# Meowuu7/equi-articulated-pose

Hardware: AMD Instinct MI355X
Metric: point-clouds/sec (4096 pts, 60 anchors) fwd+bwd (higher is better)
Workload: dtype f32; 1 GPU; 8 x 4096-pt synthetic laptop clouds per GPU, 3-block inter backbone 1->64->128->512 (NN=64,K=24,A=60), forward+backward+Adam; clouds_per_gpu=8, points=4096, anchors=60

## Files before the change

equi-articulated-pose_amd/csrc/inv_lists.hip:

```cpp
#include "common.h"

namespace {

constexpr int RT = 1024;
constexpr int MAXN = 16384;
constexpr int SORT_COMPACT = 2048;

__global__ __launch_bounds__(256) void inv_count_kernel(int per_cloud, int n, const int32_t *__restrict__ idx,
                                                        int32_t *__restrict__ counts) {
    extern __shared__ int s_hist[];
    const int bi = blockIdx.y, t = threadIdx.x;
    for (int i = t; i < n; i += 256) s_hist[i] = 0;
    __syncthreads();
    const int chunk = (per_cloud + gridDim.x - 1) / gridDim.x;
    const int beg = blockIdx.x * chunk, end = min(per_cloud, beg + chunk);
    const int32_t *src = idx + (size_t)bi * per_cloud;
    for (int e = beg + t; e < end; e += 256) {
        const int q = src[e];
        if ((unsigned)q < (unsigned)n) atomicAdd(&s_hist[q], 1);
    }
    __syncthreads();
    for (int i = t; i < n; i += 256) {
        const int v = s_hist[i];
        if (v) atomicAdd(&counts[(size_t)bi * n + i], v);
// ... 118 lines not shown
                                                          const int32_t *__restrict__ rows, const float4 *__restrict__ src,
                                                          float4 *__restrict__ dst) {
    const int bi = blockIdx.z, ci = blockIdx.y;
    const int e = blockIdx.x * 256 + threadIdx.x;
    if (e >= rcap * na4) return;
    const int r = e / na4, a = e - r * na4;
    const int q = rows[(size_t)bi * rld + r];
    float4 v = make_float4(0.f, 0.f, 0.f, 0.f);
    if (q >= 0) v = src[(((size_t)bi * c + ci) * n + q) * na4 + a];
    dst[(((size_t)bi * c + ci) * rcap + r) * na4 + a] = v;
}

__global__ __launch_bounds__(256) void rows_scatter_kernel(int c, int n, int na4, int rcap, int rld,
                                                           const int32_t *__restrict__ rows, const float4 *__restrict__ src,
                                                           float4 *__restrict__ dst) {
    const int bi = blockIdx.z, ci = blockIdx.y;
    const int e = blockIdx.x * 256 + threadIdx.x;
    if (e >= rcap * na4) return;
    const int r = e / na4, a = e - r * na4;
    const int q = rows[(size_t)bi * rld + r];
    if (q >= 0) dst[(((size_t)bi * c + ci) * n + q) * na4 + a] = src[(((size_t)bi * c + ci) * rcap + r) * na4 + a];
}

}

extern "C" int eap_inv_lists_rows(int b, int p, int n, int nn, const int32_t *idx, int32_t *counts, int32_t *rows,
                                  int32_t *off, int32_t *cnt, int32_t *n_rows, eap_stream_t stream) {
    if (b <= 0 || p <= 0 || nn <= 0 || n <= 0) return 0;
    if (n > MAXN) return eap::bad_arg("inv_lists_rows: more than 16384 support points per cloud");
    if ((long long)p * nn >= (1ll << 31)) return eap::bad_arg("inv_lists_rows: more than 2^31 entries per cloud");
    hipStream_t s = eap::S(stream);
    int e = eap::hip_fail(hipMemsetAsync(counts, 0, sizeof(int32_t) * (size_t)b * n, s), "inv_lists_rows memset");
    if (e) return e;
    const int per_cloud = p * nn;
    e = eap::run_kernel("inv_lists_rows (count)", inv_count_kernel, eap::cdiv(per_cloud, 8192), b, 1, dim3(256), sizeof(int) * n, s, per_cloud, n, idx, counts);
    if (e) return e;
    int n2 = RT;
    while (n2 < n) n2 <<= 1;
    const size_t shmem = sizeof(unsigned long long) * n2;
    return eap::run_kernel("inv_lists_rows (sort)", inv_rows_kernel, b, 1, 1, dim3(RT), shmem, s, n, n2, counts, rows, off, cnt, n_rows);
}

extern "C" int eap_inv_lists_fill(int b, int p, int n, int nn, int rcap, const int32_t *idx, const float *gx,
                                  const int32_t *rows, const int32_t *off, int32_t *ent_p, float *ent_gx,
                                  eap_stream_t stream) {
    if (b <= 0 || p <= 0 || nn <= 0 || rcap <= 0) return 0;
    if (((long long)p * nn & 3) != 0) return eap::bad_arg("inv_lists_fill: p * nn must be a multiple of 4");
    if (rcap > n) return eap::bad_arg("inv_lists_fill: rcap exceeds the number of support points");
    return eap::run_kernel("inv_lists_fill", inv_fill_kernel, rcap, b, 1, dim3(256), 0, eap::S(stream), p * nn, nn, n, n, idx, reinterpret_cast<const float4 *>(gx),
                           rows, off, ent_p, reinterpret_cast<float4 *>(ent_gx));
}

extern "C" int eap_rows_gather_f32(int b, int c, int n, int na, int rcap, int rows_ld, const int32_t *rows,
                                   const float *src, float *dst, eap_stream_t stream) {
    if (b <= 0 || c <= 0 || rcap <= 0) return 0;
    if ((na & 3) != 0) return eap::bad_arg("rows_gather: na must be a multiple of 4");
    return eap::run_kernel("rows_gather", rows_gather_kernel, eap::cdiv((long long)rcap * (na / 4), 256), c, b, dim3(256), 0, eap::S(stream), c, n, na / 4, rcap, rows_ld,
                           rows, reinterpret_cast<const float4 *>(src), reinterpret_cast<float4 *>(dst));
}

extern "C" int eap_rows_scatter_f32(int b, int c, int n, int na, int rcap, int rows_ld, const int32_t *rows,
                                    const float *src, float *dst, eap_stream_t stream) {
    if (b <= 0 || c <= 0) return 0;
    if ((na & 3) != 0) return eap::bad_arg("rows_scatter: na must be a multiple of 4");
    hipStream_t s = eap::S(stream);
    int e = eap::hip_fail(hipMemsetAsync(dst, 0, sizeof(float) * (size_t)b * c * n * na, s), "rows_scatter memset");
    if (e || rcap <= 0) return e;
    return eap::run_kernel("rows_scatter", rows_scatter_kernel, eap::cdiv((long long)rcap * (na / 4), 256), c, b, dim3(256), 0, s, c, n, na / 4, rcap, rows_ld, rows,
                           reinterpret_cast<const float4 *>(src), reinterpret_cast<float4 *>(dst));
}
```

equi-articulated-pose_amd/csrc/norm_fold.hip:

```cpp
#include <math.h>
#include <string.h>

#include "common.h"

namespace {

constexpr int WAVE = 64;

__device__ __forceinline__ double wave_sum(double v) {
#pragma unroll
    for (int m = WAVE / 2; m >= 1; m >>= 1) v += __shfl_xor(v, m, WAVE);
    return v;
}

__device__ __forceinline__ void two_row_sums(const float *__restrict__ a, const float *__restrict__ q, int parts, int lane, double &sa, double &sq) {
    sa = 0.0, sq = 0.0;
    for (int i = lane; i < parts; i += WAVE) {
        sa += (double)a[i];
        sq += (double)q[i];
    }
    sa = wave_sum(sa);
    sq = wave_sum(sq);
}

// ... 75 lines not shown
    }
}

__global__ __launch_bounds__(256) void dense_zbound_kernel(int b, int na, int rp, int p, int ldw, long cnt_stride, const float *__restrict__ colmax,
                                                           const int32_t *__restrict__ cnt, const int32_t *__restrict__ n_rows,
                                                           float *__restrict__ words) {
    const int w = blockIdx.x * blockDim.x + threadIdx.x, cloud = blockIdx.y;
    if (w >= ldw) return;
    float v = 0.f;
    if (w < na * rp / 4) {
        const int a = 4 * w / rp, r0 = 4 * w - a * rp, live = n_rows[cloud];
        const float m = colmax[(long)cloud * na + a];
#pragma unroll
        for (int j = 0; j < 4; ++j) {
            int c = r0 + j < live ? cnt[cloud * cnt_stride + r0 + j] : 0;
            c = c < 0 ? 0 : (c > p ? p : c);
            const float t = m * (float)c;
            v = j == 0 ? t : nan_max(v, t);
        }
    }
    words[(long)cloud * ldw + w] = v;
}

__global__ __launch_bounds__(256) void dense_gbound_parts_kernel(int bc, int c, int rp, int na, int ks, const float *__restrict__ W3,
                                                                 const float *__restrict__ fc4, float *__restrict__ fpart, float *__restrict__ wsum) {
    __shared__ float red[256];
    const int t = threadIdx.x, nt = blockDim.x;
    if ((int)blockIdx.x < bc) {
        const float *src = fc4 + (long)blockIdx.x * rp * na;
        const int len = rp * na;
        float m = 0.f, m1 = 0.f, m2 = 0.f, m3 = 0.f;
        int e = t;
        for (; e + 3 * nt < len; e += 4 * nt) {
            const float v0 = src[e], v1 = src[e + nt], v2 = src[e + 2 * nt], v3 = src[e + 3 * nt];
            m = nan_max(m, fabsf(v0)), m1 = nan_max(m1, fabsf(v1)), m2 = nan_max(m2, fabsf(v2)), m3 = nan_max(m3, fabsf(v3));
        }
        for (; e < len; e += nt) m = nan_max(m, fabsf(src[e]));
        m = nan_max(nan_max(m, m1), nan_max(m2, m3));
        red[t] = m;
        __syncthreads();
        if (t < na) {
            for (int g = 1; g < nt / na; ++g) m = nan_max(m, red[t + g * na]);
            fpart[(long)blockIdx.x * na + t] = m;
        }
        return;
    }
    const int oc = blockIdx.x - bc, lane = t & (WAVE - 1), wave = t / WAVE, waves = nt / WAVE;
    float m = 0.f;
    if (wave < waves)
        for (int k = wave; k < ks; k += waves) {
            const float *row = W3 + ((long)oc * ks + k) * c;
            double s = 0.0;
            for (int i = lane; i < c; i += WAVE) s += (double)fabsf(row[i]);
            m = nan_max(m, (float)wave_sum(s));
        }
    if (lane == 0 && wave < waves) red[wave] = m;
    __syncthreads();
    if (t == 0) {
        for (int g = 1; g < waves; ++g) m = nan_max(m, red[g]);
        wsum[oc] = m * 1.0001f;
    }
}

__global__ __launch_bounds__(256) void dense_gbound_kernel(int c, int na, int o, const float *__restrict__ fpart, const float *__restrict__ wsum,
                                                           float *__restrict__ bound) {
    __shared__ float red[256];
    const int t = threadIdx.x, cloud = blockIdx.x / na, a = blockIdx.x - cloud * na;
    float m = 0.f;
    for (int ch = t; ch < c; ch += 256) m = nan_max(m, fpart[((long)cloud * c + ch) * na + a]);
    red[t] = m;
    __syncthreads();
    for (int s = 128; s >= 1; s >>= 1) {
        if (t < s) red[t] = nan_max(red[t], red[t + s]);
        __syncthreads();
    }
    m = red[0];
    for (int oc = t; oc < o; oc += 256) bound[(long)blockIdx.x * o + oc] = m * wsum[oc];
}

__global__ __launch_bounds__(256) void dense_point_order_kernel(int p, int quads, const int64_t *__restrict__ order, const int4 *__restrict__ memb,
                                                                const float *__restrict__ q_xyz, int32_t *__restrict__ order32,
                                                                int4 *__restrict__ memb_out, float *__restrict__ xyz_out,
                                                                int32_t *__restrict__ pivot_pos) {
    const long i = (long)blockIdx.x * blockDim.x + threadIdx.x;
// ... 55 lines not shown
                                        const int32_t *n_rows, float *words, eap_stream_t stream) {
    if (!colmax || !cnt || !n_rows || !words) return eap::bad_arg("so3_dense_zbound: null pointer");
    if (b <= 0 || na <= 0 || rp <= 0 || p <= 0 || ldz <= 0) return eap::bad_arg("so3_dense_zbound: b, na, rp, p and ldz must be positive");
    if (rp % 4 != 0 || ldz % 4 != 0 || (long long)na * rp > ldz || cnt_stride < rp)
        return eap::bad_arg("so3_dense_zbound: rp and ldz multiples of 4, ldz >= na * rp, the row stride of cnt >= rp");
    return eap::run_kernel("so3_dense_zbound", dense_zbound_kernel, eap::cdiv(ldz / 4, 256), b, 1, dim3(256), 0, eap::S(stream), b, na, rp, p, ldz / 4,
                           (long)cnt_stride, colmax, cnt, n_rows, words);
}

extern "C" int eap_so3_dense_gplanes_bound_f32(int b, int o, int c, int na, int ks, int rp, const float *W3, const float *fc4, float *fpart,
                                               float *wsum, float *bound, eap_stream_t stream) {
    if (!W3 || !fc4 || !fpart || !wsum || !bound) return eap::bad_arg("so3_dense_gplanes_bound: null pointer");
    if (b <= 0 || o <= 0 || c <= 0 || na <= 0 || ks <= 0 || rp <= 0) return eap::bad_arg("so3_dense_gplanes_bound: every size must be positive");
    if (na > 128 || (long long)rp * na > 0x7fffffffLL || (long long)b * c > 0x7fffffffLL - o || (long long)b * na > 0x7fffffffLL)
        return eap::bad_arg("so3_dense_gplanes_bound: na <= 128, rp * na, b * c + o and b * na below 2^31");
    const int nt = 256 / na * na;
    if (int e = eap::run_kernel("so3_dense_gplanes_bound (parts)", dense_gbound_parts_kernel, (long long)b * c + o, 1, 1, dim3(nt), 0, eap::S(stream), b * c, c,
                                rp, na, ks, W3, fc4, fpart, wsum))
        return e;
    return eap::run_kernel("so3_dense_gplanes_bound", dense_gbound_kernel, (long long)b * na, 1, 1, dim3(256), 0, eap::S(stream), c, na, o, (const float *)fpart,
                           (const float *)wsum, bound);
}

extern "C" int eap_so3_dense_point_order(int b, int p, int words, const int64_t *order, const uint32_t *memb, const float *q_xyz, int32_t *order32,
                                         uint32_t *memb_out, float *xyz_out, int32_t *pivot_pos, eap_stream_t stream) {
    if (!order || !memb || !q_xyz || !order32 || !memb_out || !xyz_out || !pivot_pos) return eap::bad_arg("so3_dense_point_order: null pointer");
    if (b <= 0 || p <= 0) return eap::bad_arg("so3_dense_point_order: b and p must be positive");
    if (words != 16 && words != 32) return eap::bad_arg("so3_dense_point_order: 16 or 32 membership words per point");
    if (!aligned16(memb) || !aligned16(memb_out)) return eap::bad_arg("so3_dense_point_order: takes 16-byte aligned membership tables");
    const int quads = words / 4;
    return eap::run_kernel("so3_dense_point_order", dense_point_order_kernel, eap::cdiv((long long)p * quads, 256), b, 1, dim3(256), 0, eap::S(stream), p, quads,
                           order, reinterpret_cast<const int4 *>(memb), q_xyz, order32, reinterpret_cast<int4 *>(memb_out), xyz_out, pivot_pos);
}
```

equi-articulated-pose_amd/vgtk/_hip.py:

```python
import ctypes
import os
import re
import struct
import types
import weakref

import torch

_PKG_ROOT = os.path.abspath(os.path.join(os.path.dirname(__file__), '..'))
LIB_PATH = os.path.join(_PKG_ROOT, 'libeap_hip.so')

if not os.path.exists(LIB_PATH):
    raise ImportError(
        f'{LIB_PATH} not found: build the HIP extension first '
        '(python -c "import __graft_entry__ as g; g.build()" or make -C equi-articulated-pose_amd/csrc). '
        'This package has no CPU fallback.')

lib = ctypes.CDLL(LIB_PATH)


_HEADERS = (os.path.join(_PKG_ROOT, 'include', 'eap_hip.h'), os.path.join(os.path.dirname(_PKG_ROOT), 'include', 'eap_hip.h'))
HEADER_PATH = next((p for p in _HEADERS if os.path.exists(p)), _HEADERS[-1])

_I64 = ctypes.c_int64
# ... 706 lines not shown
         tag={'flops': 2.0 * b * o * ks * p * nn * na, 'shape': ('group_inv_perm2', b, o, p, nn, na, ks, rcap)})
    return z


def inv_lists_rows(idx, n):
    b, p, nn = idx.shape
    dev = idx.device
    counts = torch.empty(b, n, dtype=torch.int32, device=dev)
    rows, off, cnt = torch.empty_like(counts), torch.empty_like(counts), torch.empty_like(counts)
    n_rows = torch.empty(b, dtype=torch.int32, device=dev)
    call('eap_inv_lists_rows', idx, b, p, n, nn, idx, counts, rows, off, cnt, n_rows)
    return rows, off, cnt, n_rows


def inv_lists_fill(idx, gx, rows, off, rcap):
    b, p, nn = idx.shape
    n = rows.shape[1]
    ent_p = torch.empty(b, p * nn, dtype=torch.int32, device=idx.device)
    ent_gx = torch.empty(b, p * nn, 4, dtype=torch.float32, device=idx.device)
    call('eap_inv_lists_fill', idx, b, p, n, nn, int(rcap), idx, gx, rows, off, ent_p, ent_gx)
    return ent_p, ent_gx


def rows_gather(src, rows, rcap):
    b, c, n, na = src.shape
    dst = torch.empty(b, c, rcap, na, dtype=torch.float32, device=src.device)
    call('eap_rows_gather_f32', src, b, c, n, na, int(rcap), rows.stride(0), rows, src, dst)
    return dst


def rows_scatter(src, rows, n):
    b, c, rcap, na = src.shape
    dst = torch.empty(b, c, n, na, dtype=torch.float32, device=src.device)
    call('eap_rows_scatter_f32', src, b, c, n, na, int(rcap), rows.stride(0), rows, src, dst)
    return dst





def so3_dense_supported(p, na, ks, rp, o):
    return bool(abi.eap_so3_dense_supported(int(p), int(na), int(ks), int(rp), int(o)))


DENSE_MAX_ROWS = int(abi.eap_so3_dense_max_rows())
DENSE_NARROW_ROWS = 512


def _dense_wide(memb):
    return memb.shape[2] == 32
# ... 144 lines not shown
        if geo.n_rows is not None:
            rows = sum(min((int(r) + 15) & ~15, geo.rp) for r in geo.n_rows.tolist())
    return 6.0 * o * p * geo.na * geo.ks * rows


def _dense_product(direction, geo, b, o, p, ld, scale, planes, out, flops):
    call('eap_so3_dense_product_steps_f32', out, direction, b, o, p, geo.na, geo.ks, geo.rp, ld, geo.sigma, geo.n_rows, planes, scale, geo.pt, geo.kr,
         geo.mask(direction), geo.steps(direction), out, tag={'flops': flops, 'executed_f16_flops': _dense_executed_flops(geo, o, p, direction),
         'shape': ('so3_dense', direction, b, o, p, geo.na, geo.ks, geo.rp)})
    return out


def so3_dense_bwd(gy, geo, ldz=None, colmap=None, rowmax=False):
    b, o, p, na = gy.shape
    ldz = na * geo.rp if ldz is None else int(ldz)
    colmap = geo.columns(colmap)
    scale, planes = so3_dense_split(gy, rowmax=take_rowmax_hint(gy) if rowmax is False else rowmax, colmap=colmap)
    if colmap is not None:
        p = colmap.shape[1]
    z = torch.empty(b, o, geo.ks, ldz, dtype=torch.float32, device=gy.device)
    return _dense_product(0, geo, b, o, p, ldz, scale, planes, z, 2.0 * b * o * p * na * geo.ks * geo.nn)


def so3_dense_gplanes(fc4, W3, geo):
    b, c, rp, na = fc4.shape
    o = W3.shape[0] // geo.ks
    if not GPLANES or not abi.eap_so3_dense_gplanes_supported(o, c, na, geo.ks, rp):
        return None
    ft = fc4.permute(0, 3, 2, 1).contiguous()
    if NATIVE_NORM_GLUE:
        bound = so3_dense_gplanes_bound(W3, fc4, geo.ks)
    else:
        wsum = W3.abs().sum(1).view(o, geo.ks).amax(1)
        fm = fc4.abs().amax((1, 2))
        bound = (fm[:, :, None] * (wsum * 1.0001)[None, None, :]).contiguous()
    scale = torch.empty(2, b, na, o, dtype=torch.float32, device=fc4.device)
    planes = torch.empty(b * na * o * ((geo.ks * rp + 31) // 32 * 32), dtype=torch.int32, device=fc4.device)
    call('eap_so3_dense_gplanes_f32', fc4, b, o, c, na, geo.ks, rp, W3, ft, geo.n_rows, bound, scale, planes,
         tag={'flops': 0.0, 'shape': ('so3_dense_gplanes', b, o, c, na, geo.ks, rp)})
    return scale, planes


GPLANES = True


NATIVE_NORM_GLUE = True


def _f64_bits(x):
    return struct.unpack('<q', struct.pack('<d', float(x)))[0]


def norm_fold_train(ps, pq, pivot, count, gamma, beta, eps, momentum, running_mean, running_var):
    check_input(ps, pq, gamma, beta, running_mean, running_var)
    o, parts = ps.shape
    if pivot.dim() != 1 or pivot.shape[0] != o or pivot.dtype != torch.float32 or not pivot.is_cuda:
        raise RuntimeError('norm_fold_train: pivot must be a float32 device vector (any stride) of one element per channel')
    dev = ps.device
    scale, shift, beta_copy, inv_gamma = (torch.empty(o, dtype=torch.float32, device=dev) for _ in range(4))
    mean, invstd = (torch.empty(o, dtype=torch.float64, device=dev) for _ in range(2))
    call('eap_norm_fold_train_f32', ps, o, parts, max(int(pivot.stride(0)), 1), int(count), _f64_bits(eps), _f64_bits(momentum), ps, pq, pivot, gamma,
# ... 15 lines not shown
    colmax = torch.empty(b, na, dtype=torch.float32, device=dev)
    call('eap_norm_fold_bwd_f32', pg, o, parts, b, na, int(count), pg, pgx, k1, beta, inv_gamma, gmax, xmax, dgamma, dbeta, k2, k3, coef, bound, colmax)
    return dgamma, dbeta, k2, k3, coef, bound, colmax


def so3_dense_zbound(colmax, cnt, n_rows, rp, p, ldz):
    b, na = colmax.shape
    if cnt.dtype != torch.int32 or n_rows.dtype != torch.int32 or cnt.stride(1) != 1 or not n_rows.is_contiguous():
        raise RuntimeError('so3_dense_zbound: cnt and n_rows must be int32, the rows of cnt contiguous')
    words = torch.empty(b, ldz // 4, dtype=torch.float32, device=colmax.device)
    call('eap_so3_dense_zbound_f32', colmax, b, na, int(rp), int(p), int(ldz), cnt.stride(0), colmax, cnt, n_rows, words)
    return words


def so3_dense_gplanes_bound(W3, fc4, ks):
    check_input(W3, fc4)
    b, c, rp, na = fc4.shape
    o = W3.shape[0] // ks
    dev = fc4.device
    fpart = torch.empty(b, c, na, dtype=torch.float32, device=dev)
    wsum = torch.empty(o, dtype=torch.float32, device=dev)
    bound = torch.empty(b, na, o, dtype=torch.float32, device=dev)
    call('eap_so3_dense_gplanes_bound_f32', fc4, b, o, c, na, int(ks), rp, W3, fc4, fpart, wsum, bound)
    return bound


def so3_dense_point_order(order, memb, q_xyz):
    check_input(order, memb, q_xyz)
    b, p = order.shape
    order32 = torch.empty(b, p, dtype=torch.int32, device=order.device)
    memb_out, xyz_out = torch.empty_like(memb), torch.empty_like(q_xyz)
    pivot_pos = torch.empty(1, dtype=torch.int32, device=order.device)
    call('eap_so3_dense_point_order', order, b, p, memb.shape[2], order, memb, q_xyz, order32, memb_out, xyz_out, pivot_pos)
    return order32, memb_out, xyz_out, pivot_pos


def so3_dense_fwd(g, geo, p, c=0, ldg=None, out=None, col_map=None, operand=None, o=None):
    yt = _dense_fwd_yt(g, geo, p, c, ldg, operand, o)
    b, na, o = yt.shape[0], geo.na, yt.shape[2]
    if col_map is not None:
        if out is None or col_map.dtype != torch.int32 or tuple(col_map.shape) != (b, p) or not col_map.is_contiguous() or not out.is_contiguous():
            raise RuntimeError('so3_dense_fwd: col_map must be a contiguous int32 [b,p] and come with a contiguous out')
        call('eap_so3_dense_untranspose_map_f32', yt, b, o, p, na, out.shape[2], geo.columns(col_map), yt, out)
        return out
    y = torch.empty(b, o, p, na, dtype=torch.float32, device=yt.device)
    chunks = (p + 63) // 64
# ... 363 lines not shown
```

equi-articulated-pose_amd/vgtk/so3conv/functional.py:

```python
import math
import os
import weakref

import numpy as np
import torch

import vgtk
import vgtk.functional as fr
import vgtk.pc as pctk
import vgtk.spconv as zpconv
import vgtk.cuda.grouping as cuda_nn

from .. import _hip
from . import norm_fold

inter_so3conv_feat_grouping = zpconv.inter_zpconv_grouping_naive
batched_index_select = zpconv.batched_index_select
batched_index_select_other = zpconv.batched_index_select_other

MATERIALIZE_INTER_W = False

GAMMA_SIZE = 3
ROOT = vgtk.__path__[0]
Rs, R_idx, canonical_relative = fr.icosahedron_so3(GAMMA_SIZE)
# ... 954 lines not shown
    scale, shift, mean, invstd, count, slope, sync = bn
    b, o = gy.shape[0], gy.shape[1]
    gy = gy.view(b, o, -1)
    if _native_norm_bwd(gy, count, sync):
        g_bn_w, g_bn_b, k2, k3 = _hip.norm_fold_bwd(*_hip.narrow_conv_bwd_reduce(gy, x, W, scale, shift, mean, invstd, slope, partials=True), scale, count)
        return (_hip.narrow_conv_bwd_dw(gy, x, W, scale, shift, mean, invstd, k2, k3, slope) if need_w else None), g_bn_w, g_bn_b
    sg, sgx = _hip.narrow_conv_bwd_reduce(gy, x, W, scale, shift, mean, invstd, slope)
    gW = None
    if need_w:
        k2, k3 = norm_fold.backward_coefficients(scale, sg, sgx, count, True, sync)
        gW = _hip.narrow_conv_bwd_dw(gy, x, W, scale, shift, mean, invstd, k2, k3, slope)
    return gW, sgx.float(), sg.float()



def _weight_operand(W, c, ks, pad_c=None):
    o = W.shape[0]
    W2 = W.view(o, c, ks).permute(1, 0, 2).reshape(c, o * ks).contiguous()
    if pad_c is not None and pad_c != c:
        W2 = torch.cat([W2, torch.zeros(pad_c - c, o * ks, dtype=torch.float32, device=W.device)])
    return W2


def _rows_grad_from_z(z, W2, c, rp, na, ldz, anchor_major, z_bound=None, reorder=None):
    b, (pad_c, oks) = z.shape[0], W2.shape
    gFc = torch.empty(b, pad_c, ldz, dtype=torch.float32, device=z.device)
    _hip.matmul(W2, z.view(b, oks, ldz), gFc, b_bound=z_bound)
    if anchor_major:
        return gFc[:, :c, :rp * na].reshape(b, c, na, rp).transpose(2, 3)
    gFc = gFc.view(b, c, rp, na)
    return gFc if reorder is None else _hip.anchor_reorder(gFc, reorder)


def _weight_grad_rows(z, fc4, o, ks, ldz, anchor_major, reorder=None):
    b, c, rp, na = fc4.shape
    if reorder is not None:
        fc4 = _hip.anchor_reorder(fc4, reorder)
    fc = fc4.transpose(2, 3).contiguous() if anchor_major else fc4
    return _weight_grad_from_z(z, fc.view(b, c, rp * na), b, c, o, ks, rp * na, ldz)



def _backward_dense(gy, W, feats, head, geo, bn, yact, need_f, need_w):
    b, c, n, na = feats.shape
    o, ks, p, rp = W.shape[0], geo.ks, gy.shape[2], geo.rp
    if BACKWARD_LOG is not None:
        BACKWARD_LOG.append({'channels': (c, o), 'support_rows': n, 'referenced_rows_max': int(rp), 'regime': 'dense rows',
                             **({'norm': 'in the node'} if bn is not None else {})})
    ra = na * rp
    pad_c = 128 if (c == 64 and bn is not None) else c
# ... 4 lines not shown
        native = _native_norm_bwd(gy, count, sync)
        if native:
            pg, pgx, gmax, xmax = _hip.bn_act_bwd_reduce_fromy(gy, yact, beta, inv_gamma, slope, partials=True)
            g_bn_w, g_bn_b, _, _, coef, bound, colmax = _hip.norm_fold_bwd(pg, pgx, k1, count, beta, inv_gamma, gmax, xmax)
        else:
            sg, sgx, gmax, xmax = _hip.bn_act_bwd_reduce_fromy(gy, yact, beta, inv_gamma, slope)
            g_bn_w, g_bn_b = sgx.float(), sg.float()
            k2, k3 = norm_fold.backward_coefficients(k1, sg, sgx, count, True, sync)
            coef = torch.stack([k1, k2, k3, beta, inv_gamma]).contiguous()
            bound = (k1.abs()[None, :, None] * gmax + k2.abs()[None, :, None] + k3.abs()[None, :, None] * xmax).contiguous()
        z = _hip.so3_dense_bwd_bn(gy, yact, geo, ldz, coef, bound, slope)
        if ldz % 4 == 0 and rp % 4 == 0 and native:
            z_bound = (_hip.so3_dense_zbound(colmax, head.cnt, head.n_rows, rp, p, ldz).view(torch.int32), 4, 1.0)
        elif ldz % 4 == 0 and rp % 4 == 0:
            live = torch.arange(rp, device=gy.device)[None, :] < head.n_rows[:, None]
            cntf = torch.where(live, head.cnt[:, :rp], torch.zeros_like(head.cnt[:, :rp])).clamp(min=0, max=p).to(torch.float32)
            cols = bound.amax(1)[:, :, None] * cntf[:, None, :]
            words = torch.zeros(b, ldz // 4, dtype=torch.float32, device=gy.device)
            words[:, :ra // 4] = cols.view(b, na, rp // 4, 4).amax(3).view(b, ra // 4)
            z_bound = (words.view(torch.int32), 4, 1.0)
    else:
        z = _hip.so3_dense_bwd(gy, geo, ldz)
    if need_f:
        gFr = _rows_grad_from_z(z, _weight_operand(W, c, ks, pad_c), c, rp, na, ldz, True, z_bound)
        gF = _hip.rows_scatter(gFr.contiguous(), head.rows, n)
    if need_w:
        gW = _weight_grad_rows(z, _hip.rows_gather(feats, head.rows, rp), o, ks, ldz, True)
    return gF, gW, g_bn_w, g_bn_b


def _backward_dense_parts(gy, W, feats, head, pd, need_f, need_w):
    b, c, n, na = feats.shape
    o, ks, rp = W.shape[0], pd.ks, pd.rp
    ra = na * rp
    if BACKWARD_LOG is not None:
        BACKWARD_LOG.append({'channels': (c, o), 'support_rows': n, 'referenced_rows_max': int(rp), 'regime': 'dense rows', 'parts': pd.parts.n})
    ldz = _hip.dense_pitch(ra) if (c % 128 == 0 and (o * ks) % 16 == 0 and need_f) else ra
    W2 = _weight_operand(W, c, ks) if need_f else None
    fc0 = _hip.rows_gather(feats, head.rows, rp) if need_w else None
    gFr = gW = None
    rowmax = _hip.take_rowmax_hint(gy)
    for i, geo in enumerate(pd.geo):
        perm = pd.perm[i]
        z = _hip.so3_dense_bwd(gy, geo, ldz, colmap=pd.parts.col_map[i], rowmax=rowmax)
        pe = None if perm is None else perm[:, None].expand(b, c, rp, na)
        if need_f:
            t = _rows_grad_from_z(z, W2, c, rp, na, ldz, True)
            if gFr is None:
                gFr = torch.zeros(b, c, rp, na, dtype=torch.float32, device=gy.device)
            if pe is None:
# ... 762 lines not shown
```

include/eap_hip.h:

```cpp
#ifndef EAP_HIP_H
#define EAP_HIP_H

#include <stdint.h>

#ifdef __cplusplus
extern "C" {
#endif

typedef void *eap_stream_t;

const char *eap_last_error(void);
int eap_launch_dims_ok(int64_t gx, int64_t gy, int64_t gz, int bx, int by, int bz);
const char *eap_last_kernel(void);
int eap_abi_version(void);


int eap_ball_query_f32(int b, int n, int m, float radius, int nsample, const float *new_xyz,
                       const float *xyz, int32_t *idx, eap_stream_t stream);
int eap_ball_query_f64(int b, int n, int m, float radius, int nsample, const double *new_xyz,
                       const double *xyz, int32_t *idx, eap_stream_t stream);

int eap_furthest_point_sampling_f32(int b, int n, int m, const float *xyz, float *temp,
                                    int32_t *idx, eap_stream_t stream);
int eap_furthest_point_sampling_f64(int b, int n, int m, const double *xyz, double *temp,
// ... 145 lines not shown
int eap_so3_inter_group_inv_f32(int b, int o, int p, int nn, int na, int ks, int rcap, float sigma,
                                const float *gy, const int32_t *rows, const int32_t *off,
                                const int32_t *cnt, const int32_t *ent_p, const float *ent_gx,
                                const float *rk, const uint8_t *multinv, const float *anchors,
                                int identity_anchor, float *z, eap_stream_t stream);
int eap_anchor_reorder_f32(int64_t rows, int na, const float *src, const uint8_t *order, float *dst, eap_stream_t stream);
int eap_anchor_reorder_clouds_f32(int b, int64_t rows_per_cloud, int na, const float *src, const uint8_t *order,
                                  const int32_t *nonident, float *dst, eap_stream_t stream);
int eap_so3_inter_group_inv_coset_f32(int b, int o, int p, int nn, int na, int ks, int rcap, float sigma,
                                      const float *gy, const int32_t *rows, const int32_t *off, const int32_t *cnt,
                                      const int32_t *ent_p, const float *ent_gx, const float *rk, const uint8_t *multinv,
                                      const float *anchors, int identity_anchor, const uint8_t *coset_order,
                                      const uint8_t *coset_code, float *z, eap_stream_t stream);

int eap_inv_lists_rows(int b, int p, int n, int nn, const int32_t *idx, int32_t *counts, int32_t *rows,
                       int32_t *off, int32_t *cnt, int32_t *n_rows, eap_stream_t stream);
int eap_inv_lists_fill(int b, int p, int n, int nn, int rcap, const int32_t *idx, const float *gx,
                       const int32_t *rows, const int32_t *off, int32_t *ent_p, float *ent_gx,
                       eap_stream_t stream);
int eap_rows_gather_f32(int b, int c, int n, int na, int rcap, int rows_ld, const int32_t *rows,
                        const float *src, float *dst, eap_stream_t stream);
int eap_rows_scatter_f32(int b, int c, int n, int na, int rcap, int rows_ld, const int32_t *rows,
                         const float *src, float *dst, eap_stream_t stream);

int eap_so3_dense_supported(int p, int na, int ks, int rp, int o);
int eap_so3_dense_member(int b, int p, int n, int nn, int rp, int rows_ld, const int32_t *idx, const int32_t *rows,
                         const int32_t *n_rows, int32_t *slot_of, uint32_t *memb, int32_t *flags, eap_stream_t stream);
int64_t eap_so3_dense_mask_words(int b, int p, int ks, int rp, int dir);
int eap_so3_dense_masks(int b, int p, int ks, int rp, int dir, const uint32_t *memb, uint64_t *mask, eap_stream_t stream);
int eap_so3_dense_tables_f32(int b, int p, int n, int na, int ks, int rp, int rows_ld, float sigma, const float *q_xyz,
                             const float *s_xyz, const int32_t *rows, const float *rk, const float *row_rot, float *centre, float *pt,
                             float *kr, eap_stream_t stream);
int eap_so3_dense_split_f32(int b, int m, int l, int na, int seg, int64_t seg_pitch, int mapped, const int32_t *n_rows, const uint32_t *rowmax,
                            const int32_t *colmap, const float *src, float *scale, void *planes, eap_stream_t stream);
int eap_so3_dense_product_f32(int dir, int b, int o, int p, int na, int ks, int rp, int64_t ldz, float sigma, const int32_t *n_rows, const void *planes,
                              const float *scale,
                              const float *pt, const float *kr, const uint64_t *mask, float *out, eap_stream_t stream);
int eap_so3_dense_untranspose_f32(int b, int o, int p, int na, const float *yt, float *y, float *psum, float *psq, eap_stream_t stream);
int eap_so3_dense_untranspose_map_f32(int b, int o, int p, int na, int p_dst, const int32_t *map, const float *yt, float *y,
                                      eap_stream_t stream);
int eap_so3_dense_untranspose_map_stats_f32(int b, int o, int p, int na, int p_dst, const int32_t *map, const int32_t *pivot_pos, const float *yt,
                                            float *y, float *psum, float *psq, eap_stream_t stream);
int eap_so3_dense_split_bn_f32(int b, int m, int l, int l_src, int na, const uint32_t *rowbound, const int32_t *colmap, const float *grad,
                               const float *act, const float *coef, float slope, float *scale, void *planes, eap_stream_t stream);
int eap_so3_dense_untranspose_bnact_f32(int b, int o, int p, int na, int p_dst, const int32_t *map, const float *yt, const float *bn_scale,
                                        const float *bn_shift, float slope, float *y, eap_stream_t stream);
// ... 189 lines not shown

int eap_narrow_conv_segments(int64_t n);
int eap_narrow_conv_stats_f32(int b, int o, int ck, int64_t n, const float *W, const float *x, float *pivot, float *psum, float *psq,
                              eap_stream_t stream);
int eap_narrow_conv_bnact_fwd_f32(int b, int o, int ck, int64_t n, float slope, const float *W, const float *x, const float *scale,
                                  const float *shift, float *y, eap_stream_t stream);
int eap_narrow_conv_bwd_reduce_f32(int b, int o, int ck, int64_t n, float slope, const float *gy, const float *x, const float *W,
                                   const float *scale, const float *shift, const float *mean, const float *invstd, float *pg, float *pgx,
                                   eap_stream_t stream);
int eap_narrow_conv_bwd_dw_f32(int b, int o, int ck, int64_t n, float slope, const float *gy, const float *x, const float *W,
                               const float *scale, const float *shift, const float *mean, const float *invstd, const float *k2,
                               const float *k3, float *partial, float *dW, eap_stream_t stream);

int eap_norm_fold_train_f32(int o, int parts, int64_t pivot_stride, int64_t count, int64_t eps_bits, int64_t momentum_bits, const float *ps,
                            const float *pq, const float *pivot, const float *gamma, const float *beta, float *running_mean, float *running_var,
                            float *scale, float *shift, double *mean, double *invstd, float *beta_copy, float *inv_gamma, eap_stream_t stream);
int eap_norm_fold_bwd_f32(int o, int parts, int b, int na, int64_t count, const float *pg, const float *pgx, const float *k1, const float *beta,
                          const float *inv_gamma, const float *gmax, const float *xmax, float *dgamma, float *dbeta, float *k2, float *k3, float *coef,
                          float *bound, float *colmax, eap_stream_t stream);
int eap_so3_dense_zbound_f32(int b, int na, int rp, int p, int ldz, int64_t cnt_stride, const float *colmax, const int32_t *cnt,
                             const int32_t *n_rows, float *words, eap_stream_t stream);
int eap_so3_dense_gplanes_bound_f32(int b, int o, int c, int na, int ks, int rp, const float *W3, const float *fc4, float *fpart, float *wsum,
                                    float *bound, eap_stream_t stream);
int eap_so3_dense_point_order(int b, int p, int words, const int64_t *order, const uint32_t *memb, const float *q_xyz, int32_t *order32,
                              uint32_t *memb_out, float *xyz_out, int32_t *pivot_pos, eap_stream_t stream);

int eap_anchor_attn_pool_fwd_f32(int b, int c, int n, int na, float temperature, const float *x, const float *logits,
                                 float *out, float *conf, eap_stream_t stream);
int eap_anchor_attn_pool_bwd_f32(int b, int c, int n, int na, float temperature, const float *x, const float *logits,
                                 const float *g, float *dx, float *dlogits, eap_stream_t stream);
int eap_slot_masked_mean_fwd_f32(int b, int ns, int c, int n, int na, const float *x, const float *mask,
                                 const float *inv_den, float *out, eap_stream_t stream);
int eap_slot_masked_mean_bwd_f32(int b, int ns, int c, int n, int na, const float *g, const float *mask,
                                 const float *inv_den, float *dx, eap_stream_t stream);
int eap_masked_max_fwd_f32(int b, int c, int n, int na, const float *x, const float *mask, float *out, int32_t *arg,
                           eap_stream_t stream);
int eap_masked_max_bwd_f32(int b, int c, int n, int na, const float *g, const int32_t *arg, const float *mask, float *dx,
                           eap_stream_t stream);
int eap_anchor_attn_pool_wide_fwd_f32(int b, int c, int n, int na, float temperature, const float *x, const float *logits,
                                      float *out, float *conf, eap_stream_t stream);
int eap_anchor_attn_pool_wide_bwd_f32(int b, int c, int n, int na, float temperature, const float *x, const float *logits,
                                      const float *g, float *dx, float *dlogits, eap_stream_t stream);
int eap_slot_masked_mean_wide_fwd_f32(int b, int ns, int c, int n, int na, const float *x, const float *mask,
                                      const float *inv_den, float *out, eap_stream_t stream);
int eap_slot_masked_mean_wide_bwd_f32(int b, int ns, int c, int n, int na, const float *g, const float *mask,
                                      const float *inv_den, float *dx, eap_stream_t stream);
// ... 70 lines not shown
```

Before: 173.4 point-clouds/sec.

## Gather and scatter support rows directly in anchor-major layout in dense backward

```diff
diff --git a/equi-articulated-pose_amd/csrc/inv_lists.hip b/equi-articulated-pose_amd/csrc/inv_lists.hip
--- a/equi-articulated-pose_amd/csrc/inv_lists.hip
+++ b/equi-articulated-pose_amd/csrc/inv_lists.hip
@@ -164,6 +164,78 @@
     if (q >= 0) dst[(((size_t)bi * c + ci) * n + q) * na4 + a] = src[(((size_t)bi * c + ci) * rcap + r) * na4 + a];
 }
 
+constexpr int ROWS_TILE = 64;
+
+struct DivStep {
+    int q, r, dq, dr, d;
+    __device__ __forceinline__ DivStep(int e0, int d_) : q(e0 / d_), r(e0 - (e0 / d_) * d_), dq(256 / d_), dr(256 - (256 / d_) * d_), d(d_) {}
+    __device__ __forceinline__ void next() {
+        q += dq; r += dr;
+        if (r >= d) { r -= d; ++q; }
+    }
+};
+
+__device__ __forceinline__ void tile_put4(float *t, const float4 &v) { t[0] = v.x; t[1] = v.y; t[2] = v.z; t[3] = v.w; }
+__device__ __forceinline__ float4 tile_get4(const float *t) { return make_float4(t[0], t[1], t[2], t[3]); }
+
+__global__ __launch_bounds__(256) void rows_gather_am_kernel(int c, int n, int na, int rcap, int rld, const int32_t *__restrict__ rows,
+                                                             const float *__restrict__ src, float *__restrict__ dst) {
+    extern __shared__ float rows_tile[];
+    const int bi = blockIdx.z, ci = blockIdx.y, r0 = blockIdx.x * ROWS_TILE, nr = min(ROWS_TILE, rcap - r0), pitch = na + 1, na4 = na >> 2;
+    const float *s = src + ((size_t)bi * c + ci) * n * na;
+    DivStep i(threadIdx.x, na4);
+    for (int e = threadIdx.x; e < nr * na4; e += 256, i.next()) {
+        const int q = rows[(size_t)bi * rld + r0 + i.q];
+        float4 v = make_float4(0.f, 0.f, 0.f, 0.f);
+        if ((unsigned)q < (unsigned)n) v = reinterpret_cast<const float4 *>(s + (size_t)q * na)[i.r];
+        tile_put4(rows_tile + i.q * pitch + 4 * i.r, v);
+    }
+    __syncthreads();
+    float *d = dst + ((size_t)bi * c + ci) * na * rcap + r0;
+    for (int e = threadIdx.x; e < na * ROWS_TILE; e += 256) {
+        const int a = e / ROWS_TILE, rr = e - a * ROWS_TILE;
+        if (rr < nr) d[(size_t)a * rcap + rr] = rows_tile[rr * pitch + a];
+    }
+}
+
+__global__ __launch_bounds__(256) void rows_scatter_am_kernel(int c, int n, int na, int rcap, int rld, long long sB, long long ld,
+                                                              const int32_t *__restrict__ rows, const float *__restrict__ src,
+                                                              float *__restrict__ dst) {
+    extern __shared__ float rows_tile[];
+    const int bi = blockIdx.z, ci = blockIdx.y, r0 = blockIdx.x * ROWS_TILE, nr = min(ROWS_TILE, rcap - r0), pitch = na + 1, na4 = na >> 2;
+    const float *s = src + (size_t)bi * sB + (size_t)ci * ld + r0;
+    for (int e = threadIdx.x; e < na * ROWS_TILE; e += 256) {
+        const int a = e / ROWS_TILE, rr = e - a * ROWS_TILE;
+        if (rr < nr) rows_tile[rr * pitch + a] = s[(size_t)a * rcap + rr];
+    }
+    __syncthreads();
+    float *d = dst + ((size_t)bi * c + ci) * n * na;
+    DivStep i(threadIdx.x, na4);
+    for (int e = threadIdx.x; e < nr * na4; e += 256, i.next()) {
+        const int q = rows[(size_t)bi * rld + r0 + i.q];
+        if ((unsigned)q < (unsigned)n) reinterpret_cast<float4 *>(d + (size_t)q * na)[i.r] = tile_get4(rows_tile + i.q * pitch + 4 * i.r);
+    }
+}
+
+__global__ __launch_bounds__(256) void rows_gather_ft_kernel(int c, int n, int na, int rcap, int rld, const int32_t *__restrict__ rows,
+                                                             const float *__restrict__ src, float *__restrict__ dst) {
+    extern __shared__ float rows_tile[];
+    const int bi = blockIdx.y, r = blockIdx.x, pitch = na + 1, na4 = na >> 2;
+    const int q = rows[(size_t)bi * rld + r];
+    const bool live = (unsigned)q < (unsigned)n;
+    const float *s = src + ((size_t)bi * c * n + (live ? q : 0)) * na;
+    DivStep i(threadIdx.x, na4);
+    for (int e = threadIdx.x; e < c * na4; e += 256, i.next()) {
+        float4 v = make_float4(0.f, 0.f, 0.f, 0.f);
+        if (live) v = reinterpret_cast<const float4 *>(s + (size_t)i.q * n * na)[i.r];
+        tile_put4(rows_tile + i.q * pitch + 4 * i.r, v);
+    }
+    __syncthreads();
+    float *d = dst + ((size_t)bi * na * rcap + r) * c;
+    DivStep o(threadIdx.x, c);
+    for (int e = threadIdx.x; e < na * c; e += 256, o.next()) d[(size_t)o.q * rcap * c + o.r] = rows_tile[o.r * pitch + o.q];
+}
+
 }
 
 extern "C" int eap_inv_lists_rows(int b, int p, int n, int nn, const int32_t *idx, int32_t *counts, int32_t *rows,
@@ -201,6 +273,41 @@
                            rows, reinterpret_cast<const float4 *>(src), reinterpret_cast<float4 *>(dst));
 }
 
+extern "C" int eap_rows_gather_layout_f32(int b, int c, int n, int na, int rcap, int rows_ld, int layout, const int32_t *rows,
+                                          const float *src, float *dst, eap_stream_t stream) {
+    if (layout < 0 || layout > 2) return eap::bad_arg("rows_gather_layout: layout must be 0 ([b,c,rcap,na]), 1 ([b,c,na,rcap]) or 2 ([b,na,rcap,c])");
+    if (b <= 0 || c <= 0 || rcap <= 0) return 0;
+    if (rows == nullptr || src == nullptr || dst == nullptr) return eap::bad_arg("rows_gather_layout: null pointer");
+    if (n <= 0 || na <= 0 || (na & 3) != 0 || rows_ld < rcap) return eap::bad_arg("rows_gather_layout: n and na must be positive, na a multiple of 4, rows_ld >= rcap");
+    if (!eap::aligned16(src)) return eap::bad_arg("rows_gather_layout: src must be 16-byte aligned (its rows are read as 16-byte pieces)");
+    if (layout == 0) return eap_rows_gather_f32(b, c, n, na, rcap, rows_ld, rows, src, dst, stream);
+    if (layout == 1)
+        return eap::run_kernel("rows_gather (anchor-major)", rows_gather_am_kernel, eap::cdiv(rcap, ROWS_TILE), c, b, dim3(256), sizeof(float) * ROWS_TILE * (na + 1),
+                               eap::S(stream), c, n, na, rcap, rows_ld, rows, src, dst);
+    const size_t lds = sizeof(float) * (size_t)c * (na + 1);
+    if (lds > 64 * 1024) return eap::bad_arg("rows_gather_layout: layout 2 takes c * (na + 1) <= 16384 floats (one support row in LDS)");
+    return eap::run_kernel("rows_gather (channel-innermost)", rows_gather_ft_kernel, rcap, b, 1, dim3(256), lds, eap::S(stream), c, n, na, rcap, rows_ld, rows, src,
+                           dst);
+}
+
+extern "C" int eap_rows_scatter_am_f32(int b, int c, int n, int na, int rcap, int rows_ld, int64_t src_batch, int64_t src_ld, const int32_t *rows,
+                                       const float *src, float *dst, eap_stream_t stream) {
+    if (b <= 0 || c <= 0) return 0;
+    if (dst == nullptr) return eap::bad_arg("rows_scatter_am: null pointer");
+    if (n <= 0 || na <= 0 || (na & 3) != 0) return eap::bad_arg("rows_scatter_am: n and na must be positive, na a multiple of 4");
+    if (!eap::aligned16(dst)) return eap::bad_arg("rows_scatter_am: dst must be 16-byte aligned (its rows are written as 16-byte pieces)");
+    hipStream_t s = eap::S(stream);
+    if (rcap > 0) {
+        if (rows == nullptr || src == nullptr) return eap::bad_arg("rows_scatter_am: null pointer");
+        if (rows_ld < rcap || src_ld < (int64_t)na * rcap || (src_ld & 3) != 0 || src_batch < (int64_t)c * src_ld)
+            return eap::bad_arg("rows_scatter_am: rows_ld >= rcap, src_ld >= na * rcap and a multiple of 4, src_batch >= c * src_ld");
+    }
+    int e = eap::hip_fail(hipMemsetAsync(dst, 0, sizeof(float) * (size_t)b * c * n * na, s), "rows_scatter_am memset");
+    if (e || rcap <= 0) return e;
+    return eap::run_kernel("rows_scatter (anchor-major)", rows_scatter_am_kernel, eap::cdiv(rcap, ROWS_TILE), c, b, dim3(256), sizeof(float) * ROWS_TILE * (na + 1), s, c,
+                           n, na, rcap, rows_ld, (long long)src_batch, (long long)src_ld, rows, src, dst);
+}
+
 extern "C" int eap_rows_scatter_f32(int b, int c, int n, int na, int rcap, int rows_ld, const int32_t *rows,
                                     const float *src, float *dst, eap_stream_t stream) {
     if (b <= 0 || c <= 0) return 0;
diff --git a/equi-articulated-pose_amd/csrc/norm_fold.hip b/equi-articulated-pose_amd/csrc/norm_fold.hip
--- a/equi-articulated-pose_amd/csrc/norm_fold.hip
+++ b/equi-articulated-pose_amd/csrc/norm_fold.hip
@@ -121,6 +121,25 @@
     words[(long)cloud * ldw + w] = v;
 }
 
+__device__ __forceinline__ void gbound_wsum(int oc, int c, int ks, const float *__restrict__ W3, float *__restrict__ wsum, float *red) {
+    const int t = threadIdx.x, nt = blockDim.x;
+    const int lane = t & (WAVE - 1), wave = t / WAVE, waves = nt / WAVE;
+    float m = 0.f;
+    if (wave < waves)
+        for (int k = wave; k < ks; k += waves) {
+            const float *row = W3 + ((long)oc * ks + k) * c;
+            double s = 0.0;
+            for (int i = lane; i < c; i += WAVE) s += (double)fabsf(row[i]);
+            m = nan_max(m, (float)wave_sum(s));
+        }
+    if (lane == 0 && wave < waves) red[wave] = m;
+    __syncthreads();
+    if (t == 0) {
+        for (int g = 1; g < waves; ++g) m = nan_max(m, red[g]);
+        wsum[oc] = m * 1.0001f;
+    }
+}
+
 __global__ __launch_bounds__(256) void dense_gbound_parts_kernel(int bc, int c, int rp, int na, int ks, const float *__restrict__ W3,
                                                                  const float *__restrict__ fc4, float *__restrict__ fpart, float *__restrict__ wsum) {
     __shared__ float red[256];
@@ -144,21 +163,39 @@
         }
         return;
     }
-    const int oc = blockIdx.x - bc, lane = t & (WAVE - 1), wave = t / WAVE, waves = nt / WAVE;
-    float m = 0.f;
-    if (wave < waves)
-        for (int k = wave; k < ks; k += waves) {
-            const float *row = W3 + ((long)oc * ks + k) * c;
-            double s = 0.0;
-            for (int i = lane; i < c; i += WAVE) s += (double)fabsf(row[i]);
-            m = nan_max(m, (float)wave_sum(s));
-        }
-    if (lane == 0 && wave < waves) red[wave] = m;
+    gbound_wsum(blockIdx.x - bc, c, ks, W3, wsum, red);
+}
+
+__global__ __launch_bounds__(256) void dense_gbound_ft_parts_kernel(int bna, int c, int rp, int ks, const float *__restrict__ W3,
+                                                                    const float *__restrict__ ft, float *__restrict__ fmax, float *__restrict__ wsum) {
+    __shared__ float red[256];
+    const int t = threadIdx.x;
+    if ((int)blockIdx.x >= bna) {
+        gbound_wsum(blockIdx.x - bna, c, ks, W3, wsum, red);
+        return;
+    }
+    const float *src = ft + (long)blockIdx.x * rp * c;
+    const long len = (long)rp * c;
+    float m = 0.f, m1 = 0.f, m2 = 0.f, m3 = 0.f;
+    long e = t;
+    for (; e + 3 * 256 < len; e += 4 * 256) {
+        const float v0 = src[e], v1 = src[e + 256], v2 = src[e + 512], v3 = src[e + 768];
+        m = nan_max(m, fabsf(v0)), m1 = nan_max(m1, fabsf(v1)), m2 = nan_max(m2, fabsf(v2)), m3 = nan_max(m3, fabsf(v3));
+    }
+    for (; e < len; e += 256) m = nan_max(m, fabsf(src[e]));
+    red[t] = nan_max(nan_max(m, m1), nan_max(m2, m3));
     __syncthreads();
-    if (t == 0) {
-        for (int g = 1; g < waves; ++g) m = nan_max(m, red[g]);
-        wsum[oc] = m * 1.0001f;
-    }
+    for (int s = 128; s >= 1; s >>= 1) {
+        if (t < s) red[t] = nan_max(red[t], red[t + s]);
+        __syncthreads();
+    }
+    if (t == 0) fmax[blockIdx.x] = red[0];
+}
+
+__global__ __launch_bounds__(256) void dense_gbound_ft_kernel(long total, int o, const float *__restrict__ fmax, const float *__restrict__ wsum,
+                                                              float *__restrict__ bound) {
+    const long i = (long)blockIdx.x * 256 + threadIdx.x;
+    if (i < total) bound[i] = fmax[i / o] * wsum[i % o];
 }
 
 __global__ __launch_bounds__(256) void dense_gbound_kernel(int c, int na, int o, const float *__restrict__ fpart, const float *__restrict__ wsum,
@@ -260,6 +297,20 @@
                            (const float *)wsum, bound);
 }
 
+extern "C" int eap_so3_dense_gplanes_bound_ft_f32(int b, int o, int c, int na, int ks, int rp, const float *W3, const float *ft, float *fmax,
+                                                  float *wsum, float *bound, eap_stream_t stream) {
+    if (!W3 || !ft || !fmax || !wsum || !bound) return eap::bad_arg("so3_dense_gplanes_bound_ft: null pointer");
+    if (b <= 0 || o <= 0 || c <= 0 || na <= 0 || ks <= 0 || rp <= 0) return eap::bad_arg("so3_dense_gplanes_bound_ft: every size must be positive");
+    if ((long long)b * na > 0x7fffffffLL - o || (long long)b * na * o > 0x7fffffffLL * 256)
+        return eap::bad_arg("so3_dense_gplanes_bound_ft: b * na + o below 2^31, b * na * o below 2^39");
+    if (int e = eap::run_kernel("so3_dense_gplanes_bound_ft (parts)", dense_gbound_ft_parts_kernel, (long long)b * na + o, 1, 1, dim3(256), 0, eap::S(stream), b * na,
+                                c, rp, ks, W3, ft, fmax, wsum))
+        return e;
+    const long total = (long)b * na * o;
+    return eap::run_kernel("so3_dense_gplanes_bound_ft", dense_gbound_ft_kernel, eap::cdiv(total, 256), 1, 1, dim3(256), 0, eap::S(stream), total, o,
+                           (const float *)fmax, (const float *)wsum, bound);
+}
+
 extern "C" int eap_so3_dense_point_order(int b, int p, int words, const int64_t *order, const uint32_t *memb, const float *q_xyz, int32_t *order32,
                                          uint32_t *memb_out, float *xyz_out, int32_t *pivot_pos, eap_stream_t stream) {
     if (!order || !memb || !q_xyz || !order32 || !memb_out || !xyz_out || !pivot_pos) return eap::bad_arg("so3_dense_point_order: null pointer");
diff --git a/equi-articulated-pose_amd/vgtk/_hip.py b/equi-articulated-pose_amd/vgtk/_hip.py
--- a/equi-articulated-pose_amd/vgtk/_hip.py
+++ b/equi-articulated-pose_amd/vgtk/_hip.py
@@ -752,10 +752,28 @@
     return ent_p, ent_gx
 
 
-def rows_gather(src, rows, rcap):
+ROWS_LAYOUTS = {'rows': 0, 'anchor_major': 1, 'channel_last': 2}
+
+
+def rows_gather(src, rows, rcap, layout='rows'):
     b, c, n, na = src.shape
-    dst = torch.empty(b, c, rcap, na, dtype=torch.float32, device=src.device)
-    call('eap_rows_gather_f32', src, b, c, n, na, int(rcap), rows.stride(0), rows, src, dst)
+    rcap = int(rcap)
+    if layout == 'rows':
+        dst = torch.empty(b, c, rcap, na, dtype=torch.float32, device=src.device)
+        call('eap_rows_gather_f32', src, b, c, n, na, rcap, rows.stride(0), rows, src, dst)
+        return dst
+    shape = (b, c, na, rcap) if layout == 'anchor_major' else (b, na, rcap, c)
+    dst = torch.empty(shape, dtype=torch.float32, device=src.device)
+    call('eap_rows_gather_layout_f32', src, b, c, n, na, rcap, rows.stride(0), ROWS_LAYOUTS[layout], rows, src, dst)
+    return dst
+
+
+def rows_scatter_am(src, c, rcap, na, rows, n):
+    b, ld = src.shape[0], src.stride(1)
+    if src.dim() != 3 or src.stride(2) != 1 or src.dtype != torch.float32:
+        raise RuntimeError('rows_scatter_am: src must be a float32 [b, rows, columns] with contiguous columns')
+    dst = torch.empty(b, c, n, na, dtype=torch.float32, device=src.device)
+    call('eap_rows_scatter_am_f32', src, b, int(c), int(n), int(na), int(rcap), rows.stride(0), src.stride(0), ld, rows, src, dst)
     return dst
 
 
@@ -946,21 +964,31 @@
     return _dense_product(0, geo, b, o, p, ldz, scale, planes, z, 2.0 * b * o * p * na * geo.ks * geo.nn)
 
 
-def so3_dense_gplanes(fc4, W3, geo):
-    b, c, rp, na = fc4.shape
+def so3_dense_gplanes_takes(o, c, na, ks, rp):
+    return bool(GPLANES and abi.eap_so3_dense_gplanes_supported(o, c, na, ks, rp))
+
+
+def so3_dense_gplanes(fc4, W3, geo, ft=None):
+    if fc4 is None:
+        b, na, rp, c = ft.shape
+    else:
+        b, c, rp, na = fc4.shape
     o = W3.shape[0] // geo.ks
-    if not GPLANES or not abi.eap_so3_dense_gplanes_supported(o, c, na, geo.ks, rp):
+    if not so3_dense_gplanes_takes(o, c, na, geo.ks, rp):
         return None
-    ft = fc4.permute(0, 3, 2, 1).contiguous()
-    if NATIVE_NORM_GLUE:
-        bound = so3_dense_gplanes_bound(W3, fc4, geo.ks)
+    if fc4 is None:
+        bound = so3_dense_gplanes_bound_ft(W3, ft, geo.ks)
     else:
-        wsum = W3.abs().sum(1).view(o, geo.ks).amax(1)
-        fm = fc4.abs().amax((1, 2))
-        bound = (fm[:, :, None] * (wsum * 1.0001)[None, None, :]).contiguous()
-    scale = torch.empty(2, b, na, o, dtype=torch.float32, device=fc4.device)
-    planes = torch.empty(b * na * o * ((geo.ks * rp + 31) // 32 * 32), dtype=torch.int32, device=fc4.device)
-    call('eap_so3_dense_gplanes_f32', fc4, b, o, c, na, geo.ks, rp, W3, ft, geo.n_rows, bound, scale, planes,
+        ft = fc4.permute(0, 3, 2, 1).contiguous()
+        if NATIVE_NORM_GLUE:
+            bound = so3_dense_gplanes_bound(W3, fc4, geo.ks)
+        else:
+            wsum = W3.abs().sum(1).view(o, geo.ks).amax(1)
+            fm = fc4.abs().amax((1, 2))
+            bound = (fm[:, :, None] * (wsum * 1.0001)[None, None, :]).contiguous()
+    scale = torch.empty(2, b, na, o, dtype=torch.float32, device=ft.device)
+    planes = torch.empty(b * na * o * ((geo.ks * rp + 31) // 32 * 32), dtype=torch.int32, device=ft.device)
+    call('eap_so3_dense_gplanes_f32', ft, b, o, c, na, geo.ks, rp, W3, ft, geo.n_rows, bound, scale, planes,
          tag={'flops': 0.0, 'shape': ('so3_dense_gplanes', b, o, c, na, geo.ks, rp)})
     return scale, planes
 
@@ -1022,6 +1050,18 @@
     wsum = torch.empty(o, dtype=torch.float32, device=dev)
     bound = torch.empty(b, na, o, dtype=torch.float32, device=dev)
     call('eap_so3_dense_gplanes_bound_f32', fc4, b, o, c, na, int(ks), rp, W3, fc4, fpart, wsum, bound)
+    return bound
+
+
+def so3_dense_gplanes_bound_ft(W3, ft, ks):
+    check_input(W3, ft)
+    b, na, rp, c = ft.shape
+    o = W3.shape[0] // ks
+    dev = ft.device
+    fmax = torch.empty(b * na, dtype=torch.float32, device=dev)
+    wsum = torch.empty(o, dtype=torch.float32, device=dev)
+    bound = torch.empty(b, na, o, dtype=torch.float32, device=dev)
+    call('eap_so3_dense_gplanes_bound_ft_f32', ft, b, o, c, na, int(ks), rp, W3, ft, fmax, wsum, bound)
     return bound
 
 
diff --git a/equi-articulated-pose_amd/vgtk/so3conv/functional.py b/equi-articulated-pose_amd/vgtk/so3conv/functional.py
--- a/equi-articulated-pose_amd/vgtk/so3conv/functional.py
+++ b/equi-articulated-pose_amd/vgtk/so3conv/functional.py
@@ -1000,10 +1000,16 @@
     return W2
 
 
-def _rows_grad_from_z(z, W2, c, rp, na, ldz, anchor_major, z_bound=None, reorder=None):
+def _rows_grad_gemm(z, W2, ldz, z_bound=None):
     b, (pad_c, oks) = z.shape[0], W2.shape
     gFc = torch.empty(b, pad_c, ldz, dtype=torch.float32, device=z.device)
     _hip.matmul(W2, z.view(b, oks, ldz), gFc, b_bound=z_bound)
+    return gFc
+
+
+def _rows_grad_from_z(z, W2, c, rp, na, ldz, anchor_major, z_bound=None, reorder=None):
+    b = z.shape[0]
+    gFc = _rows_grad_gemm(z, W2, ldz, z_bound)
     if anchor_major:
         return gFc[:, :c, :rp * na].reshape(b, c, na, rp).transpose(2, 3)
     gFc = gFc.view(b, c, rp, na)
@@ -1054,10 +1060,11 @@
     else:
         z = _hip.so3_dense_bwd(gy, geo, ldz)
     if need_f:
-        gFr = _rows_grad_from_z(z, _weight_operand(W, c, ks, pad_c), c, rp, na, ldz, True, z_bound)
-        gF = _hip.rows_scatter(gFr.contiguous(), head.rows, n)
+        gFc = _rows_grad_gemm(z, _weight_operand(W, c, ks, pad_c), ldz, z_bound)
+        gF = _hip.rows_scatter_am(gFc, c, rp, na, head.rows, n)
     if need_w:
-        gW = _weight_grad_rows(z, _hip.rows_gather(feats, head.rows, rp), o, ks, ldz, True)
+        fc = _hip.rows_gather(feats, head.rows, rp, layout='anchor_major')
+        gW = _weight_grad_from_z(z, fc.view(b, c, ra), b, c, o, ks, ra, ldz)
     return gF, gW, g_bn_w, g_bn_b
 
 
diff --git a/include/eap_hip.h b/include/eap_hip.h
--- a/include/eap_hip.h
+++ b/include/eap_hip.h
@@ -191,6 +191,10 @@
                         const float *src, float *dst, eap_stream_t stream);
 int eap_rows_scatter_f32(int b, int c, int n, int na, int rcap, int rows_ld, const int32_t *rows,
                          const float *src, float *dst, eap_stream_t stream);
+int eap_rows_gather_layout_f32(int b, int c, int n, int na, int rcap, int rows_ld, int layout, const int32_t *rows,
+                               const float *src, float *dst, eap_stream_t stream);
+int eap_rows_scatter_am_f32(int b, int c, int n, int na, int rcap, int rows_ld, int64_t src_batch, int64_t src_ld, const int32_t *rows,
+                            const float *src, float *dst, eap_stream_t stream);
 
 int eap_so3_dense_supported(int p, int na, int ks, int rp, int o);
 int eap_so3_dense_member(int b, int p, int n, int nn, int rp, int rows_ld, const int32_t *idx, const int32_t *rows,
@@ -426,6 +430,8 @@
                              const int32_t *n_rows, float *words, eap_stream_t stream);
 int eap_so3_dense_gplanes_bound_f32(int b, int o, int c, int na, int ks, int rp, const float *W3, const float *fc4, float *fpart, float *wsum,
                                     float *bound, eap_stream_t stream);
+int eap_so3_dense_gplanes_bound_ft_f32(int b, int o, int c, int na, int ks, int rp, const float *W3, const float *ft, float *fmax, float *wsum,
+                                       float *bound, eap_stream_t stream);
 int eap_so3_dense_point_order(int b, int p, int words, const int64_t *order, const uint32_t *memb, const float *q_xyz, int32_t *order32,
                               uint32_t *memb_out, float *xyz_out, int32_t *pivot_pos, eap_stream_t stream);
 
```

Result: no change. 174.1 point-clouds/sec, median of 6 (+0.4%).
